# markusmoenig/Rusterix

Measured on AMD Instinct MI355X. Metric: Mpixels/s (+ ms/frame) on rasterize_map @3840x2160, 1/2/4/8 MI355X vs CPU, higher is better.
Workload: dtype f32; 1 GPU; map scene (minigame room), 3840x2160, 16 point lights, Nearest sampling, fence cut-outs, 2D logo rectangle; UV jitter absent in the reference snapshot; triangles_3d=27, light_math=relaxed

## Files before the change

### rusterix_amd/csrc/rxr_kernels.hip

```cpp
#ifndef RXR_JIT
#include <hip/hip_runtime.h>

#include <cstdlib>
#include <cstring>

#include "rxr_launch.h"
#include "rxr_route.h"
#endif

#define TS_DESC_VALID 0x80000000u

#include "rxr_device.h"
#include "rxr_exact_math.h"
#include "rxr_project.h"
#include "rxr_vm.h"

#ifndef RXR_VM_WAVES_PER_SIMD
#define RXR_VM_WAVES_PER_SIMD 6
#endif
#ifndef RXR_VEK_FUSED_MATVEC
#define RXR_VEK_FUSED_MATVEC 1
#endif

#ifndef RXR_PHASE_TIMING
// ... 312 lines not shown
    }
    return 1.0f;
}

__device__ __forceinline__ bool mapmini_is_visible(const rxr_linedef *ld, uint32_t n, float ax, float ay, float bx, float by) {
    for (uint32_t i = 0; i < n; ++i) {
        const rxr_linedef seg = uniform_record(ld, i);
        float b1x = seg.start[0], b1y = seg.start[1], b2x = seg.end[0], b2y = seg.end[1];
        float d = (bx - ax) * (b2y - b1y) - (by - ay) * (b2x - b1x);
        if (d == 0.0f) continue;
        float u = ((b1x - ax) * (b2y - b1y) - (b1y - ay) * (b2x - b1x)) / d;
        float v = ((b1x - ax) * (by - ay) - (b1y - ay) * (bx - ax)) / d;
        if ((u >= 0.0f && u <= 1.0f) && (v >= 0.0f && v <= 1.0f)) return false;
    }
    return true;
}

__device__ __forceinline__ uint32_t pack4(uint32_t r, uint32_t g, uint32_t b, uint32_t a) {
    return r | (g << 8) | (b << 16) | (a << 24);
}

__device__ __forceinline__ float grid_mul_dist(float delta, float value) {
    return fabsf(value - delta * roundf(value / delta));
}
__device__ __forceinline__ uint32_t grid_shade(const RasterParams &P, uint32_t px, uint32_t py) {
    const float grid = P.bg_grid[0], sub_div = P.bg_grid[1];
    const float pos_x = ((float)px / P.fwidth) * P.fwidth, pos_y = ((float)py / P.fheight) * P.fheight;
    const float origin_x = P.fwidth / 2.0f + P.bg_grid[2], origin_y = P.fheight / 2.0f + P.bg_grid[3];
    const float ao_x = roundf(origin_x - 0.5f) + 0.5f, ao_y = roundf(origin_y - 0.5f) + 0.5f;
    const float rel_x = pos_x - ao_x, rel_y = pos_y - ao_y;
    const float dist_x = grid_mul_dist(grid, rel_x), dist_y = grid_mul_dist(grid, rel_y);
    const uint32_t line = pack4(f32_to_u8_saturated(0.15f), f32_to_u8_saturated(0.15f), f32_to_u8_saturated(0.15f), f32_to_u8_saturated(1.0f));
    const uint32_t sub_line = pack4(f32_to_u8_saturated(0.11f), f32_to_u8_saturated(0.11f), f32_to_u8_saturated(0.11f), f32_to_u8_saturated(1.0f));
    const uint32_t bg = pack4(f32_to_u8_saturated(0.05f), f32_to_u8_saturated(0.05f), f32_to_u8_saturated(0.05f), f32_to_u8_saturated(1.0f));
    if (fminf(dist_x, dist_y) <= 1.0f * 0.5f) return line;
    const float dtf_x = fabsf(rel_x - grid * floorf(rel_x / grid)), dtf_y = fabsf(rel_y - grid * floorf(rel_y / grid));
    const float sub_size = grid / roundf(sub_div);
    float sd_x = grid_mul_dist(sub_size, dtf_x), sd_y = grid_mul_dist(sub_size, dtf_y);
    const float rc_x = roundf(dist_x / sub_size), rc_y = roundf(dist_y / sub_size);
    const float extra = grid - sub_size * sub_div;
    if (rc_x == sub_div) sd_x = sd_x + extra;
    if (rc_y == sub_div) sd_y = sd_y + extra;
    if (fminf(sd_x, sd_y) <= 1.0f * 0.5f) return sub_line;
    return bg;
}

__device__ __forceinline__ void fragment_uv(const TriShade &S, float alpha, float beta, float gamma, float &u, float &v) {
    float iu = S.u0w * alpha + S.u1w * beta + S.u2w * gamma;
    float iv = S.v0w * alpha + S.v1w * beta + S.v2w * gamma;
    float irw = S.iw0 * alpha + S.iw1 * beta + S.iw2 * gamma;
    rxm::div2(iu, iv, irw, u, v);
}

__device__ __forceinline__ const uint32_t *texel_base(const RasterParams &P, const DevTexDesc &d) {
    unsigned long long ft = (unsigned long long)P.frame_texels, rt = (unsigned long long)P.texels;
    asm volatile("" : "+v"(ft), "+v"(rt));
    typedef const uint32_t __attribute__((address_space(1))) *global_words;
    return (const uint32_t *)(global_words)((d.all_opaque & 2u) ? ft : rt);
}

__device__ __forceinline__ uint32_t terrain_texel(const RasterParams &P, const DevBatch &B, float wx, float wy) {
    const ChunkRange cr = P.chunks[B.chunk];
    const DevTexDesc d = P.tex[B.tex];
    float local_x = (wx / 1.0f) - (float)cr.origin_x;
    float local_y = (wy / 1.0f) - (float)cr.origin_y;
    float pixel_x = local_x * (float)cr.pixels_per_tile;
    float pixel_y = local_y * (float)cr.pixels_per_tile;
    uint32_t px = sat_u32(rclamp(floorf(pixel_x), 0.0f, (float)d.w - 1.0f));
    uint32_t py = sat_u32(rclamp(floorf(pixel_y), 0.0f, (float)d.h - 1.0f));
    px = min(px, d.w - 1u);
    py = min(py, d.h - 1u);
    return texel_base(P, d)[d.offset + py * d.w + px];
}

__device__ __forceinline__ float brush_blend(const RasterParams &P, f3 world, bool &inside) {
    const float dist = mag3(sub3(world, mk3(P.brush_pos[0], P.brush_pos[1], P.brush_pos[2])));
    inside = dist < P.brush_radius;
    const float normalized = dist / P.brush_radius;
    const float falloff = rclamp(P.brush_falloff, 0.001f, 1.0f);
    const float fade = rclamp((1.0f - normalized) / falloff, 0.0f, 1.0f);
    return 0.2f + 0.6f * fade;
}
__device__ __forceinline__ uint32_t brush_over_texel(const RasterParams &P, uint32_t texel, f3 world) {
    bool inside;
    const float blend = brush_blend(P, world, inside);
    if (!inside) return texel;
    uint32_t out = texel & 0xFF000000u;
#pragma unroll
    for (int i = 0; i < 3; ++i) {
        const float c = (float)((texel >> (8 * i)) & 0xFFu);
        out |= sat_u8(fminf(c * (1.0f - blend) + 255.0f * blend, 255.0f)) << (8 * i);
    }
    return out;
}

template <Level LV> inline constexpr LevelFeatures feat = level_features(LV);

template <Level LV, bool UNIFORM = false>
__device__ __forceinline__ uint32_t batch_texel(const RasterParams &P, const DevBatch &B, float u, float v, float wx, float wy, const f3 *world3 = nullptr) {
    if constexpr (!UNIFORM && !feat<LV>.chunk) {
        static_assert(__builtin_offsetof(DevBatch, tex) == 16 && __builtin_offsetof(DevBatch, pixel) == 20 && __builtin_offsetof(DevBatch, repeat_mode) == 24, "one 16-byte load");
        const uint4 hw = *reinterpret_cast<const uint4 *>(&B.tex);
        int32_t tex = (int32_t)hw.x;
        uint32_t pixel = hw.y, repeat = hw.z;
        asm volatile("" : "+v"(tex), "+v"(pixel), "+v"(repeat));
        if (tex < 0) return pixel;
        const uint4 raw = *reinterpret_cast<const uint4 *>(&P.tex[tex]);
        DevTexDesc d{raw.x, raw.y, raw.z, raw.w};
        asm volatile("" : "+v"(d.offset), "+v"(d.w), "+v"(d.h), "+v"(d.all_opaque));
        return sample_texture(d, texel_base(P, d), u, v, P.sample_mode, repeat);
    }
    if (B.tex < 0) return B.pixel;
    if constexpr (feat<LV>.chunk) {
        if (B.flags & DB_TERRAIN) {
            uint32_t t = terrain_texel(P, B, wx, wy);
            if (P.has_brush && world3) t = brush_over_texel(P, t, *world3);
            return t;
        }
    }
    if constexpr (UNIFORM) {
        const DevTexDesc d = uniform_record(P.tex, (uint32_t)B.tex);
        return sample_texture(d, texel_base(P, d), u, v, P.sample_mode, B.repeat_mode);
    } else {
        const uint4 raw = *reinterpret_cast<const uint4 *>(&P.tex[B.tex]);
        DevTexDesc d{raw.x, raw.y, raw.z, raw.w};
        asm volatile("" : "+v"(d.offset), "+v"(d.w), "+v"(d.h), "+v"(d.all_opaque));
        static_assert(sizeof(DevTexDesc) == 16, "one 16-byte load");
        return sample_texture(d, texel_base(P, d), u, v, P.sample_mode, B.repeat_mode);
    }
}

struct Frag {
    f3 world, normal, view_dir, base, lit;
    float opacity;
    uint32_t alpha_bits;
    float rough, metal;
    f3 emis;
};

__device__ __forceinline__ f3 screen_to_world_exact(const RasterParams &P, float fx, float fy, float z) {
    float vx, vy, vz, vw, wx, wy, wz, ww;
    const float x_ndc = 2.0f * rxm::div1_known(fx, P.fwidth, true) - 1.0f;
    const float y_ndc = 1.0f - 2.0f * rxm::div1_known(fy, P.fheight, true);
    mat4_mul(P.inv_proj, x_ndc, y_ndc, z, 1.0f, vx, vy, vz, vw);
    rxm::div3_self(vx, vy, vz, vw, vx, vy, vz, vw);
    mat4_mul(P.inv_view, vx, vy, vz, vw, wx, wy, wz, ww);
    return mk3(wx, wy, wz);
}

template <Level LV, bool RL = false>
__device__ __forceinline__ void shade3d_begin(const RasterParams &P, const TriShade &S, uint32_t batch_id, float alpha, float beta,
                                              float z, float fx, float fy, Frag &F, bool have_flags = false, uint32_t known_flags = 0u) {
    const DevBatch &B = P.batches3d[batch_id];
    const uint32_t b_flags = have_flags ? known_flags : B.flags;
    float gamma = 1.0f - alpha - beta;
    float u, v;
    fragment_uv(S, alpha, beta, gamma, u, v);

    bool relaxed_world = RL && !feat<LV>.chunk && !feat<LV>.programs && !P.any_occluders;
    f3 world;
    if (relaxed_world) {
        float vx, vy, vz, vw, wx, wy, wz, ww;
        mat4_mul(P.inv_proj, fmaf(fx, P.ndc_sx, -1.0f), fmaf(fy, P.ndc_sy, 1.0f), z, 1.0f, vx, vy, vz, vw);
        relaxed_world = rxm::wave_all(rxm::in_window(vw));
        if (relaxed_world) {
            const float rw = __builtin_amdgcn_rcpf(vw);
            mat4_mul(P.inv_view, vx * rw, vy * rw, vz * rw, 1.0f, wx, wy, wz, ww);
            world = mk3(wx, wy, wz);
        }
    }
    if (!relaxed_world) world = screen_to_world_exact(P, fx, fy, z);
    f3 cam = mk3(P.cam[0], P.cam[1], P.cam[2]);
    f3 view_dir, normal;
    bool relaxed_normals = false;
    if constexpr (RL && !feat<LV>.programs) {
        const bool has_n = (b_flags & DB_HAS_NORMALS) != 0u;
        const f3 vd = sub3(cam, world);
        f3 ni = mk3(0.0f, 0.0f, 0.0f);
        if (has_n) {
            f3 n0 = mk3(S.n0[0], S.n0[1], S.n0[2]), n1 = mk3(S.n1[0], S.n1[1], S.n1[2]), n2 = mk3(S.n2[0], S.n2[1], S.n2[2]);
            ni = add3(add3(scale3(n0, alpha), scale3(n1, beta)), scale3(n2, gamma));
        }
        const float vm2 = fmaf(vd.z, vd.z, fmaf(vd.y, vd.y, vd.x * vd.x)), nm2 = fmaf(ni.z, ni.z, fmaf(ni.y, ni.y, ni.x * ni.x));
        const float vinv = __builtin_amdgcn_rsqf(vm2), ninv = __builtin_amdgcn_rsqf(nm2);
        const float dnv = fmaf(ni.z, vd.z, fmaf(ni.y, vd.y, ni.x * vd.x)) * (vinv * ninv);
        float guard = P.rl_flip_guard;
        if (relaxed_world) guard = fmaf(1e-5f * vinv, __builtin_fabsf(world.x) + __builtin_fabsf(world.y) + __builtin_fabsf(world.z), guard);
        relaxed_normals = rxm::wave_all(rxm::sq_in_window(vm2) && (!has_n || (rxm::sq_in_window(nm2) && __builtin_fabsf(dnv) >= guard)));
        if (relaxed_normals) {
            view_dir = scale3(vd, vinv);
            normal = has_n ? scale3(ni, dnv < 0.0f ? -ninv : ninv) : mk3(__builtin_nanf(""), __builtin_nanf(""), __builtin_nanf(""));
        }
    }
    if (!relaxed_normals) {
        if (relaxed_world) world = screen_to_world_exact(P, fx, fy, z);
        view_dir = norm3_fast(sub3(cam, world));
        if (b_flags & DB_HAS_NORMALS) {
            f3 n0 = mk3(S.n0[0], S.n0[1], S.n0[2]), n1 = mk3(S.n1[0], S.n1[1], S.n1[2]), n2 = mk3(S.n2[0], S.n2[1], S.n2[2]);
            normal = norm3_z(add3(add3(scale3(n0, alpha), scale3(n1, beta)), scale3(n2, gamma)));
            if (dot3(normal, view_dir) < 0.0f) normal = neg3(normal);
        } else {
            normal = mk3(0.0f, 0.0f, 0.0f);
        }
    }

    uint32_t texel;
    bool desc_in_record = false;
    if constexpr (!feat<LV>.chunk || !feat<LV>.programs) desc_in_record = rxm::wave_all((S.pad[1] & TS_DESC_VALID) != 0u);
    if (desc_in_record) {
        const uint32_t p0 = S.pad[0], p1 = S.pad[1];
        const DevTexDesc d{p0, p1 & 0x1FFFu, (p1 >> 13) & 0x1FFFu, (p1 >> 28) & 3u};
        texel = sample_texture(d, texel_base(P, d), u, v, P.sample_mode, (p1 >> 26) & 3u);
    } else texel = batch_texel<LV>(P, B, u, v, world.x, world.z, &world);
    const float INV_255 = 1.0f / 255.0f;
    f3 base = mk3(srgb_to_linear_fast((float)(texel & 0xFFu) * INV_255), srgb_to_linear_fast((float)((texel >> 8) & 0xFFu) * INV_255),
                  srgb_to_linear_fast((float)((texel >> 16) & 0xFFu) * INV_255));
    F.opacity = rxm::div1_known((float)(texel >> 24), 255.0f, true);
    F.alpha_bits = texel & 0xFF000000u;
    if (feat<LV>.chunk && B.baked_plus1) {
        const DevTexDesc &baked = P.tex[B.baked_plus1 - 1u];
        uint32_t bt = sample_texture(baked, texel_base(P, baked), u, v, P.sample_mode, B.repeat_mode);
        base = mk3(srgb_to_linear_fast((float)(bt & 0xFFu) * INV_255), srgb_to_linear_fast((float)((bt >> 8) & 0xFFu) * INV_255),
                   srgb_to_linear_fast((float)((bt >> 16) & 0xFFu) * INV_255));
        F.opacity = (float)(bt >> 24) * INV_255;
    }
    float rough = 0.5f, metal = 0.0f;
    if constexpr (feat<LV>.programs) {
        if (B.program_plus1) {
            rxvm::IO io;
            rxvm::io_defaults(io);
            io.color = rxvm::mk(base.x, base.y, base.z);
            io.opacity.x = F.opacity;
            io.normal = rxvm::mk(normal.x, normal.y, normal.z);
            io.roughness.x = 0.5f;
            io.metallic.x = 0.0f;
            io.uv.x = u / 4.0f;
            io.uv.y = v / 4.0f;
            io.hitpoint = rxvm::mk(world.x, world.y, world.z);
            io.time = rxvm::splat(P.time);
            if constexpr (feat<LV>.inline_site) rxvm::shade_inline<feat<LV>.ssp>(P, B.program_plus1 - 1u, io, rxvm::stack_block());
            else rxvm::shade_call<feat<LV>.ssp>(P, B.program_plus1 - 1u, io);
            base = mk3(io.color.x, io.color.y, io.color.z);
            normal = mk3(io.normal.x, io.normal.y, io.normal.z);
            rough = rclamp(io.roughness.x, 0.0f, 1.0f);
            metal = rclamp(io.metallic.x, 0.0f, 1.0f);
            F.opacity = io.opacity.x;
            F.emis = mk3(io.emissive.x, io.emissive.y, io.emissive.z);
        }
    }

    if (!relaxed_normals) normal = norm3_z(normal);

    f3 lit = mk3(0.0f, 0.0f, 0.0f);
    float occlusion;
    static_assert(__builtin_offsetof(DevBatch, ambient) == 32 && __builtin_offsetof(DevBatch, chunk) == 44, "one 16-byte load");
    const uint4 amb_chunk = *reinterpret_cast<const uint4 *>(&B.ambient[0]);
    float amb0 = __uint_as_float(amb_chunk.x), amb1 = __uint_as_float(amb_chunk.y), amb2 = __uint_as_float(amb_chunk.z);
    int32_t b_chunk = (int32_t)amb_chunk.w;
    asm volatile("" : "+v"(amb0), "+v"(amb1), "+v"(amb2), "+v"(b_chunk));
    if (b_chunk >= 0) {
        ChunkRange cr = P.chunks[b_chunk];
        occlusion = get_occlusion(P.occluders, cr.occ_first, cr.occ_count, world.x, world.z);
    } else {
        occlusion = get_occlusion(P.occluders, 0, P.n_occluders, world.x, world.z);
    }
    float hemi = 0.5f * (normal.y + 1.0f);
    f3 kd = scale3(scale3(base, 1.0f - metal), 1.0f - 0.04f);
    if (occlusion > 0.0f) {
        if (P.flags & RXR_FLAG_HAS_AMBIENT) {
            lit = add3(lit, scale3(mul3(mk3(P.ambient[0], P.ambient[1], P.ambient[2]), kd), hemi));
        }
        if ((P.flags & RXR_FLAG_HAS_SUN) && P.day_factor > 0.0f) {
            f3 ldir = norm3(neg3(mk3(P.sun_dir[0], P.sun_dir[1], P.sun_dir[2])));
            float df = fmaxf(P.day_factor, 0.0f);
            lit = add3(lit, shade_fast_brdf(base, rough, metal, normal, view_dir, ldir, mk3(df, df, df), fmaxf(dot3(normal, ldir), 0.0f)));
        }
        lit = scale3(lit, occlusion);
    }
    lit = add3(lit, scale3(mul3(mk3(amb0, amb1, amb2), kd), hemi));
    F.world = world;
    F.normal = normal;
    F.view_dir = view_dir;
    F.base = base;
    F.lit = lit;
    F.rough = rough;
    F.metal = metal;
}

template <Level LV, bool RL = false>
__device__ __forceinline__ void shade3d_lights(const RasterParams &P, bool hit, Frag &F) {
    const unsigned long long hitmask = __ballot(hit);
    if (hitmask == 0ull) return;
    const int lane = (int)(threadIdx.x & 63u);
    const int src = __ffsll((long long)hitmask) - 1;
    const f3 c = mk3(__int_as_float(__builtin_amdgcn_readlane(__float_as_int(F.world.x), src)),
                     __int_as_float(__builtin_amdgcn_readlane(__float_as_int(F.world.y), src)),
                     __int_as_float(__builtin_amdgcn_readlane(__float_as_int(F.world.z), src)));
    const float r = hit ? mag3_bound(sub3(F.world, c)) : 0.0f;
    const bool can_cull = __ballot(hit && !(r < __builtin_huge_valf())) == 0ull;
    const float rmax = rxm::wave_max_nonneg(r);
    const float rough = feat<LV>.programs ? F.rough : 0.5f, metal = feat<LV>.programs ? F.metal : 0.0f;
    f3 rl_kd = mk3(0.0f, 0.0f, 0.0f), rl_f = rl_kd;
    float rl_shininess = 1.0f;
    if constexpr (RL && !feat<LV>.programs) {
        rl_kd = scale3(F.base, 1.0f - 0.04f);
        rl_shininess = 6.0f;
        const float om = 1.0f - rclamp(fmaxf(dot3(F.normal, F.view_dir), 0.0f), 0.0f, 1.0f);
        const float fs = 0.04f + (1.0f - 0.04f) * (om * om * om * om * om);
        rl_f = mk3(fs, fs, fs);
    } else if constexpr (RL) {
        const float tm = rclamp(metal, 0.0f, 1.0f);
        const f3 f0 = mk3(fmaf(tm, F.base.x - 0.04f, 0.04f), fmaf(tm, F.base.y - 0.04f, 0.04f), fmaf(tm, F.base.z - 0.04f, 0.04f));
        rl_kd = scale3(scale3(F.base, 1.0f - metal), 1.0f - fmaxf(f0.x, fmaxf(f0.y, f0.z)));
        rl_shininess = rclamp(2.0f / fmaxf(rough * rough, 1e-4f) - 2.0f, 1.0f, 2048.0f);
        const float om = 1.0f - rclamp(fmaxf(dot3(F.normal, F.view_dir), 0.0f), 0.0f, 1.0f);
        rl_f = add3(f0, scale3(sub3(mk3(1.0f, 1.0f, 1.0f), f0), om * om * om * om * om));
    }

    for (uint32_t base_i = 0; base_i < P.n_lights; base_i += 64u) {
        const uint32_t mine = base_i + (uint32_t)lane;
        bool cand = mine < P.n_lights;
        float ss_rcp = 0.0f;
        bool ss_ok = false;
        unsigned long long ss_ok_mask = 0ull;
        unsigned long long fast_mask = 0ull;
        if constexpr (RL) {
            bool fast = false;
            if (cand) {
                const float4 *lf4 = reinterpret_cast<const float4 *>(&P.lights_fast[mine]);
                const float4 head = lf4[0], tail = lf4[2];
                f3 lpos = mk3(head.x, head.y, head.z);
                float endd = tail.x;
                asm volatile("" : "+v"(lpos.x), "+v"(lpos.y), "+v"(lpos.z), "+v"(endd));
                const uint32_t kind = __float_as_uint(tail.y);
                fast = __float_as_uint(head.w) != 0u;
                if (can_cull && kind) {
                    float dcl = mag3_bound(sub3(c, lpos));
                    float margin = 1e-3f * (dcl + rmax + fabsf(endd)) + 1e-6f;
                    if (dcl - rmax > endd + margin) cand = false;
                }
            }
            fast_mask = __ballot(cand && fast);
            if (__ballot(cand && !fast)) {
                if (cand && !fast) {
                    const float ssd = P.lights[mine].start_distance - P.lights[mine].end_distance;
                    ss_ok = rxm::in_window(ssd);
                    ss_rcp = rxm::rcp_refined(ssd);
                }
                ss_ok_mask = __ballot(ss_ok);
            }
        } else {
            if (cand) {
                const float ssd = P.lights[mine].start_distance - P.lights[mine].end_distance;
                ss_ok = rxm::in_window(ssd);
                ss_rcp = rxm::rcp_refined(ssd);
            }
            ss_ok_mask = __ballot(ss_ok);
            if (cand && can_cull) {
                const rxr_light &L = P.lights[mine];
                if (L.light_type == RXR_LIGHT_POINT || L.light_type == RXR_LIGHT_SPOT || L.light_type == RXR_LIGHT_AREA ||
                    L.light_type == RXR_LIGHT_DAYLIGHT) {
                    float dcl = mag3_bound(sub3(c, mk3(L.position[0], L.position[1], L.position[2])));
                    float margin = 1e-3f * (dcl + rmax + fabsf(L.end_distance)) + 1e-6f;
                    if (dcl - rmax > L.end_distance + margin) cand = false;
                }
            }
        }
        unsigned long long todo = __ballot(cand);
        while (todo) {
            const int li_lane = __ffsll((long long)todo) - 1;
            const uint32_t li = base_i + (uint32_t)li_lane;
            todo &= todo - 1ull;
            float ss_r = 0.0f;
            bool ss_fast = false;
            if constexpr (!RL) {
                ss_r = __int_as_float(__builtin_amdgcn_readlane(__float_as_int(ss_rcp), li_lane));
                ss_fast = (ss_ok_mask >> li_lane) & 1ull;
            }
            if (!hit) continue;
            if constexpr (RL) {
                if ((fast_mask >> li_lane) & 1ull) {
                    const LightFast LF = uniform_record_x8(P.lights_fast, li);
                    const f3 d = sub3(mk3(LF.pos[0], LF.pos[1], LF.pos[2]), F.world);
                    const float m2 = fmaf(d.z, d.z, fmaf(d.y, d.y, d.x * d.x));
                    if (rxm::wave_all(rxm::sq_in_window(m2))) {
                        const float inv = __builtin_amdgcn_rsqf(m2);
                        const float t = __builtin_amdgcn_fmed3f(fmaf(m2 * inv, LF.ss_r, LF.c0), 0.0f, 1.0f);
                        const float ss = t * t * fmaf(-2.0f, t, 3.0f);
                        const float ndl = __builtin_amdgcn_fmed3f(fmaf(F.normal.z, d.z, fmaf(F.normal.y, d.y, F.normal.x * d.x)) * inv, 0.0f, 1.0f);
                        const f3 hu = mk3(fmaf(d.x, inv, F.view_dir.x), fmaf(d.y, inv, F.view_dir.y), fmaf(d.z, inv, F.view_dir.z));
                        const float hh = fmaf(hu.z, hu.z, fmaf(hu.y, hu.y, hu.x * hu.x));
                        const float ndh = __builtin_amdgcn_fmed3f(fmaf(F.normal.z, hu.z, fmaf(F.normal.y, hu.y, F.normal.x * hu.x)) * __builtin_amdgcn_rsqf(hh), 0.0f, 1.0f);
                        float spec;
                        if constexpr (!feat<LV>.programs) {
                            const float ndh2 = ndh * ndh;
                            spec = ndh2 * ndh2 * ndh2;
                        } else {
                            spec = __builtin_amdgcn_exp2f(rl_shininess * __builtin_amdgcn_logf(ndh));
                        }
                        const float s = ss * ndl * ndl;
                        F.lit.x = fmaf(fmaf(rl_f.x, spec, rl_kd.x), LF.cfi[0] * s, F.lit.x);
                        F.lit.y = fmaf(fmaf(rl_f.y, spec, rl_kd.y), LF.cfi[1] * s, F.lit.y);
                        F.lit.z = fmaf(fmaf(rl_f.z, spec, rl_kd.z), LF.cfi[2] * s, F.lit.z);
                        continue;
                    }
                }
            }
            if constexpr (RL) {
                ss_r = __int_as_float(__builtin_amdgcn_readlane(__float_as_int(ss_rcp), li_lane));
                ss_fast = (ss_ok_mask >> li_lane) & 1ull;
            }
            const rxr_light L = uniform_record(P.lights, li);
            const f3 lp = mk3(L.position[0], L.position[1], L.position[2]);
            f3 incoming, ldir;
            if (L.light_type == RXR_LIGHT_POINT) {
                if (!L.emitting) continue;
                f3 d = sub3(lp, F.world);
                float distance;
                ldir = norm3_fast(d, distance);
                if (distance >= L.end_distance) continue;
                float intensity = L.intensity;
                if (!(distance <= L.start_distance)) {
                    const float sn = distance - L.end_distance, sd = L.start_distance - L.end_distance;
                    float q;
                    if (ss_fast && rxm::wave_all(rxm::in_window(sn))) q = rxm::div_chain(sn, sd, ss_r);
                    else q = sn / sd;
                    const float t = rclamp(q, 0.0f, 1.0f);
                    intensity = L.intensity * (t * t * (3.0f - 2.0f * t));
                }
                incoming = apply_flicker(L, intensity, P.hash_anim);
            } else {
                if (!light_color_at(L, F.world, P.hash_anim, false, incoming)) continue;
                ldir = norm3_fast(sub3(lp, F.world));
            }
            const float n_dot_l = fmaxf(dot3(F.normal, ldir), 0.0f);
            f3 radiance;
            if (L.light_type == RXR_LIGHT_AMBIENT || L.light_type == RXR_LIGHT_AMBIENT_DAYLIGHT || L.light_type == RXR_LIGHT_DAYLIGHT) {
                radiance = incoming;
            } else {
                radiance = scale3(incoming, n_dot_l);
            }
            float rough_g = rough, metal_g = metal;
            if constexpr (RL) asm volatile("" : "+v"(rough_g), "+v"(metal_g));
            F.lit = add3(F.lit, shade_fast_brdf<RL>(F.base, rough_g, metal_g, F.normal, F.view_dir, ldir, radiance, n_dot_l));
        }
    }
}

template <Level LV, bool RL = false>
__device__ __forceinline__ uint32_t shade3d_end(const Frag &F) {
    f3 lit = F.lit;
    if constexpr (feat<LV>.programs) lit = add3(lit, F.emis);
    uint32_t alpha;
    if constexpr (feat<LV>.chunk || feat<LV>.programs) alpha = f32_to_u8_saturated(F.opacity) << 24;
    else alpha = F.alpha_bits;
    if constexpr (RL) {
        const float sx = __builtin_amdgcn_sqrtf(lit.x), sy = __builtin_amdgcn_sqrtf(lit.y), sz = __builtin_amdgcn_sqrtf(lit.z);
        return pack4(f32_to_u8_saturated(1.055f * sx - 0.055f * sx * sx), f32_to_u8_saturated(1.055f * sy - 0.055f * sy * sy),
                     f32_to_u8_saturated(1.055f * sz - 0.055f * sz * sz), 0u) | alpha;
    }
    return pack4(f32_to_u8_saturated(linear_to_srgb_fast(lit.x)), f32_to_u8_saturated(linear_to_srgb_fast(lit.y)),
                 f32_to_u8_saturated(linear_to_srgb_fast(lit.z)), 0u) | alpha;
}

template <Level LV>
__device__ __forceinline__ uint32_t shade3d_opacity(const RasterParams &P, const TriShade &S, uint32_t batch_id, float alpha, float beta,
                                                    float z, float fx, float fy) {
    const DevBatch &B = P.batches3d[batch_id];
    float gamma = 1.0f - alpha - beta;
    float u, v;
    fragment_uv(S, alpha, beta, gamma, u, v);
    float wx = 0.0f, wy = 0.0f, wz = 0.0f;
    if ((feat<LV>.chunk && (B.flags & DB_TERRAIN)) || (feat<LV>.programs && B.program_plus1)) {
        float x_ndc = 2.0f * (fx / P.fwidth) - 1.0f;
        float y_ndc = 1.0f - 2.0f * (fy / P.fheight);
        float vx, vy, vz, vw, ww;
        mat4_mul(P.inv_proj, x_ndc, y_ndc, z, 1.0f, vx, vy, vz, vw);
        vx = vx / vw;
        vy = vy / vw;
        vz = vz / vw;
        vw = vw / vw;
        mat4_mul(P.inv_view, vx, vy, vz, vw, wx, wy, wz, ww);
    }
    const f3 world3 = mk3(wx, wy, wz);
    uint32_t texel = batch_texel<LV>(P, B, u, v, wx, wz, &world3);
    const float INV_255 = 1.0f / 255.0f;
    float r = srgb_to_linear_fast((float)(texel & 0xFFu) * INV_255);
    float g = srgb_to_linear_fast((float)((texel >> 8) & 0xFFu) * INV_255);
    float b = srgb_to_linear_fast((float)((texel >> 16) & 0xFFu) * INV_255);
    float opacity = byte_over_255(texel >> 24);
    if constexpr (feat<LV>.programs) {
        if (B.program_plus1) {
            rxvm::IO io;
            rxvm::io_defaults(io);
            io.color = rxvm::mk(r, g, b);
            io.opacity.x = opacity;
            io.uv.x = u / 4.0f;
            io.uv.y = v / 4.0f;
            io.hitpoint = rxvm::mk(wx, wy, wz);
            io.time = rxvm::splat(P.time);
            io.roughness.x = 0.5f;
            io.metallic.x = 0.0f;
            rxvm::shade_call<feat<LV>.ssp>(P, B.program_plus1 - 1u, io);
            r = io.color.x;
            g = io.color.y;
            b = io.color.z;
            opacity = io.opacity.x;
        }
    }
    return pack4(f32_to_u8_saturated(linear_to_srgb_fast(r)), f32_to_u8_saturated(linear_to_srgb_fast(g)),
                 f32_to_u8_saturated(linear_to_srgb_fast(b)), f32_to_u8_saturated(opacity));
}

template <Level LV>
__device__ __forceinline__ uint32_t fragment2d(const RasterParams &P, const Prim2D &T, const DevBatch &B, uint32_t px, uint32_t py,
                                               float fx, float fy, uint32_t dst) {
    float acx = T.v2x - T.v0x, acy = T.v2y - T.v0y;
    float abx = T.v1x - T.v0x, aby = T.v1y - T.v0y;
    float apx = fx - T.v0x, apy = fy - T.v0y;
    float pcx = T.v2x - fx, pcy = T.v2y - fy;
    float pbx = T.v1x - fx, pby = T.v1y - fy;
    float area = acx * aby - acy * abx;
    float w0 = (pcx * pby - pcy * pbx) / area;
    float w1 = (acx * apy - acy * apx) / area;
    float w2 = 1.0f - w0 - w1;
    float u = T.u0 * w0 + T.u1 * w1 + T.u2 * w2;
    float v = T.v0 * w0 + T.v1 * w1 + T.v2 * w2;

    float gx = ((float)px - P.fwidth / 2.0f) - (P.translationd2[0] - P.fwidth / 2.0f);
    float gy = ((float)py - P.fheight / 2.0f) - (P.translationd2[1] - P.fheight / 2.0f);
    float wx = gx / P.scaled2, wy = gy / P.scaled2;

    uint32_t texel = batch_texel<LV, true>(P, B, u, v, wx, wy);
    if constexpr (feat<LV>.programs) {
        if (B.program_plus1 && P.programs[B.program_plus1 - 1u].shade_entry != 0xFFFFFFFFu) {
            const float INV_255 = 1.0f / 255.0f;
            rxvm::IO io;
            rxvm::io_defaults(io);
            io.uv.x = u / 4.0f;
            io.uv.y = v / 4.0f;
            io.color = rxvm::mk((float)(texel & 0xFFu) * INV_255, (float)((texel >> 8) & 0xFFu) * INV_255, (float)((texel >> 16) & 0xFFu) * INV_255);
            io.hitpoint.x = wx;
            io.hitpoint.y = wy;
            io.time = rxvm::splat(P.time);
            io.roughness.x = 0.5f;
            io.metallic.x = 0.0f;
            rxvm::shade_call<feat<LV>.ssp>(P, B.program_plus1 - 1u, io);
            texel = pack4(f32_to_u8_saturated(io.color.x), f32_to_u8_saturated(io.color.y), f32_to_u8_saturated(io.color.z), 255u);
        }
    }
    uint32_t tr = texel & 0xFFu, tg = (texel >> 8) & 0xFFu, tb = (texel >> 16) & 0xFFu, ta = texel >> 24;

    if (((B.flags & DB_RECEIVES_LIGHT) && P.any_lights) || (P.flags & RXR_FLAG_HAS_AMBIENT)) {
        float acc0 = 0.0f, acc1 = 0.0f, acc2 = 0.0f;
        uint32_t occ_first = 0, occ_count = P.n_occluders;
        if (B.chunk >= 0) {
            ChunkRange cr = P.chunks[B.chunk];
            occ_first = cr.occ_first;
            occ_count = cr.occ_count;
        }
        if (P.flags & RXR_FLAG_HAS_AMBIENT) {
            float occlusion = get_occlusion(P.occluders, occ_first, occ_count, wx, wy);
            acc0 += P.ambient[0] * occlusion;
            acc1 += P.ambient[1] * occlusion;
            acc2 += P.ambient[2] * occlusion;
        }
        for (uint32_t li = 0; li < P.n_lights; ++li) {
            const rxr_light L = uniform_record(P.lights, li);
            f3 lc;
            if (!light_color_at(L, mk3(wx, 0.0f, wy), P.hash_anim, true, lc)) continue;
            bool visible = true;
            if (L.light_type == RXR_LIGHT_AMBIENT_DAYLIGHT) {
                float occlusion = get_occlusion(P.occluders, occ_first, occ_count, wx, wy);
                lc = scale3(lc, occlusion);
            }
            if (L.light_type != RXR_LIGHT_AMBIENT && L.light_type != RXR_LIGHT_AMBIENT_DAYLIGHT &&
                !mapmini_is_visible(P.linedefs, P.n_linedefs, wx, wy, L.position[0], L.position[2]))
                visible = false;
            if (visible) {
                acc0 += lc.x;
                acc1 += lc.y;
                acc2 += lc.z;
            }
        }
        acc0 = rclamp(acc0, 0.0f, 1.0f);
        acc1 = rclamp(acc1, 0.0f, 1.0f);
        acc2 = rclamp(acc2, 0.0f, 1.0f);
        tr = sat_u8(rclamp((byte_over_255(tr) * acc0) * 255.0f, 0.0f, 255.0f));
        tg = sat_u8(rclamp((byte_over_255(tg) * acc1) * 255.0f, 0.0f, 255.0f));
        tb = sat_u8(rclamp((byte_over_255(tb) * acc2) * 255.0f, 0.0f, 255.0f));
    }

    if (ta == 255u) return pack4(tr, tg, tb, ta);
    float src_alpha = byte_over_255(ta);
    float dst_alpha = 1.0f - src_alpha;
    uint32_t dr = dst & 0xFFu, dg = (dst >> 8) & 0xFFu, db = (dst >> 16) & 0xFFu, da = dst >> 24;
    uint32_t orr = sat_u8(((float)tr * src_alpha) + ((float)dr * dst_alpha));
    uint32_t og = sat_u8(((float)tg * src_alpha) + ((float)dg * dst_alpha));
    uint32_t ob = sat_u8(((float)tb * src_alpha) + ((float)db * dst_alpha));
    uint32_t oa = (P.flags & RXR_FLAG_PRESERVE_TRANSPARENCY) ? max(da, ta) : 255u;
    return pack4(orr, og, ob, oa);
}

__device__ __forceinline__ uint32_t miss_brush_preview(const RasterParams &P, uint32_t px, uint32_t py) {
    const float ndc_x = 2.0f * ((float)px / P.fwidth) - 1.0f;
    const float ndc_y = 1.0f - 2.0f * ((float)py / P.fheight);
    float nx, ny, nz, nw, fx_, fy_, fz_, fw_;
    mat4_mul(P.inv_proj, ndc_x, ndc_y, -1.0f, 1.0f, nx, ny, nz, nw);
    mat4_mul(P.inv_proj, ndc_x, ndc_y, 1.0f, 1.0f, fx_, fy_, fz_, fw_);
    nx = nx / nw; ny = ny / nw; nz = nz / nw; nw = nw / nw;
    fx_ = fx_ / fw_; fy_ = fy_ / fw_; fz_ = fz_ / fw_; fw_ = fw_ / fw_;
    float ox, oy, oz, ow, tx, ty, tz, tw;
    mat4_mul(P.inv_view, nx, ny, nz, nw, ox, oy, oz, ow);
    mat4_mul(P.inv_view, fx_, fy_, fz_, fw_, tx, ty, tz, tw);
    const f3 origin = mk3(ox, oy, oz);
    const f3 dir = norm3(sub3(mk3(tx, ty, tz), origin));
    float c = 0.0f;
    if (fabsf(dir.y) > 1e-5f) {
        const float t = -origin.y / dir.y;
        if (t > 0.0f) {
            bool inside;
            const float blend = brush_blend(P, add3(origin, scale3(dir, t)), inside);
            if (inside) c = fminf(0.0f * (1.0f - blend) + blend, 1.0f);
        }
    }
    const uint32_t g = f32_to_u8_saturated(c);
    return pack4(g, g, g, f32_to_u8_saturated(1.0f));
}

__device__ __forceinline__ bool bin_range(const RasterParams &P, uint32_t min_x, uint32_t max_x, uint32_t min_y, uint32_t max_y,
                                          uint32_t &bx0, uint32_t &bx1, uint32_t &l0, uint32_t &l1) {
    if (!(min_x < max_x && min_y < max_y) || P.tiles_y == 0) return false;
    bx0 = min_x / RXR_TILE_W;
    bx1 = (max_x - 1) / RXR_TILE_W;
    uint32_t g0 = min_y / RXR_TILE_H, g1 = (max_y - 1) / RXR_TILE_H;
    if (g1 < P.tile_y0) return false;
    l0 = g0 <= P.tile_y0 ? 0u : (g0 - P.tile_y0 + P.tile_stride - 1u) / P.tile_stride;
    l1 = (g1 - P.tile_y0) / P.tile_stride;
    if (l1 >= P.tiles_y) l1 = P.tiles_y - 1u;
    return l0 <= l1;
}

__device__ __forceinline__ bool make_setup(const RasterParams &P, uint32_t t, TriSetup &S, TriShade &H) {
    uint32_t lo = 0, hi = P.n_batches3d;
    const bool have_info = P.tri_info != nullptr;
    uint2 info = make_uint2(0u, 0u);
    if (have_info) {
        info = P.tri_info[t];
        lo = info.x;
    } else {
        while (hi - lo > 1) {
            uint32_t mid = (lo + hi) >> 1;
            if (P.batch_tri_base[mid] <= t) lo = mid;
            else hi = mid;
        }
    }
    if (P.mesh_live && t - P.batch_tri_base[lo] >= P.mesh_live[lo]) {
        S.bx = S.by = 0u;
        return false;
    }
    const bool own_edges = P.pm_meshes != nullptr;
    const bool host_edgeless = P.edge_vis3d != nullptr;
    rxr_edges E;
    if (!own_edges && !host_edgeless) E = P.edges[t];
    const uint32_t ix0 = P.idx[3 * (size_t)t + 0], ix1 = P.idx[3 * (size_t)t + 1], ix2 = P.idx[3 * (size_t)t + 2];
    const DevBatch B = P.batches3d[lo];
    const uint32_t vbase = have_info ? info.y : B.vert_base;
    if (own_edges) {
        const DevMesh &M = P.pm_meshes[lo];
        const uint32_t local = t - P.batch_tri_base[lo];
        const bool evis = local < M.n_tris ? P.pm_edge_vis[M.tin_base + local] != 0 : true;
        E = edges_from_vertices(M.cull_mode, evis, P.pv[ix0 + vbase], P.pv[ix1 + vbase], P.pv[ix2 + vbase]);
    } else if (host_edgeless) {
        E = edges_from_vertices(B.mode, P.edge_vis3d[t] != 0u, P.pv[ix0 + vbase], P.pv[ix1 + vbase], P.pv[ix2 + vbase]);
    }

    bool skip = (B.flags & DB_SKIP) != 0;
    if (P.dev_bbox) {
        const DevBBox bb = P.dev_bbox[lo];
        auto dec = [](uint32_t e) { return __uint_as_float((e & 0x80000000u) ? (e ^ 0x80000000u) : ~e); };
        float bx = dec(bb.min_x), by = dec(bb.min_y), bw = dec(bb.max_x) - bx, bh = dec(bb.max_y) - by;
        bool keep = bx < (float)P.width && (bx + bw) > 0.0f && by < (float)P.height && (by + bh) > 0.0f;
        skip = skip || !keep;
    }
    if (!E.visible || skip) {
        S.bx = S.by = 0u;
        return false;
    }

    const uint32_t i0 = ix0 + vbase, i1 = ix1 + vbase, i2 = ix2 + vbase;
    float4 v0 = P.pv[i0], v1 = P.pv[i1], v2 = P.pv[i2];

#pragma unroll
    for (int k = 0; k < 3; ++k) {
        S.ea[k] = E.a[k];
        S.eb[k] = E.b[k];
        S.ec[k] = E.c[k];
    }
    S.v0x = v0.x; S.v0y = v0.y; S.v1x = v1.x; S.v1y = v1.y; S.v2x = v2.x; S.v2y = v2.y;
    {
        float acx = v2.x - v0.x, acy = v2.y - v0.y, abx = v1.x - v0.x, aby = v1.y - v0.y;
        S.area = acx * aby - acy * abx;
    }
    S.iz0 = 1.0f / v0.z;
    S.iz1 = 1.0f / v1.z;
    S.iz2 = 1.0f / v2.z;
    S.batch = lo;
    S.bflags = B.flags;
    S.profile_id = B.profile_id;

    H.iw0 = 1.0f / v0.w;
    H.iw1 = 1.0f / v1.w;
    H.iw2 = 1.0f / v2.w;
    float2 uv0 = P.uv[i0], uv1 = P.uv[i1], uv2 = P.uv[i2];
    H.u0w = uv0.x / v0.w; H.u1w = uv1.x / v1.w; H.u2w = uv2.x / v2.w;
    H.v0w = uv0.y / v0.w; H.v1w = uv1.y / v1.w; H.v2w = uv2.y / v2.w;
    if (B.flags & DB_HAS_NORMALS) {
#pragma unroll
        for (int k = 0; k < 3; ++k) {
            H.n0[k] = P.nrm[3 * (size_t)i0 + k];
            H.n1[k] = P.nrm[3 * (size_t)i1 + k];
            H.n2[k] = P.nrm[3 * (size_t)i2 + k];
        }
    } else {
#pragma unroll
        for (int k = 0; k < 3; ++k) H.n0[k] = H.n1[k] = H.n2[k] = 0.0f;
    }
    H.pad[0] = H.pad[1] = 0;
    if (B.tex >= 0 && !(B.flags & DB_TERRAIN) && B.repeat_mode < 4u) {
        const DevTexDesc d = P.tex[B.tex];
        if (d.w - 1u < 8191u && d.h - 1u < 8191u) {
            H.pad[0] = d.offset;
            H.pad[1] = TS_DESC_VALID | d.w | (d.h << 13) | (B.repeat_mode << 26) | ((d.all_opaque & 3u) << 28);
        }
    }
    if (P.sample_mode != RXR_SAMPLE_NEAREST && B.tex >= 0 && !(S.bflags & (DB_ALPHA_TEST | DB_FULL_ALPHA | DB_OPACITY_LIST))) {
        const float t9[9] = {H.iw0, H.iw1, H.iw2, H.u0w, H.u1w, H.u2w, H.v0w, H.v1w, H.v2w};
        bool risky = false;
#pragma unroll
        for (int k = 0; k < 9; ++k) risky = risky || !(__builtin_fabsf(t9[k]) < __builtin_huge_valf());
        const float lo = fminf(__builtin_fabsf(H.iw0), fminf(__builtin_fabsf(H.iw1), __builtin_fabsf(H.iw2)));
        const float hi = fmaxf(__builtin_fabsf(H.iw0), fmaxf(__builtin_fabsf(H.iw1), __builtin_fabsf(H.iw2)));
        const bool same_sign = (H.iw0 > 0.0f && H.iw1 > 0.0f && H.iw2 > 0.0f) || (H.iw0 < 0.0f && H.iw1 < 0.0f && H.iw2 < 0.0f);
        risky = risky || !same_sign || !(hi <= lo * 1048576.0f);
#ifndef RXR_TEST_NO_NAN_UV_RULE
        if (risky) S.bflags |= DB_ALPHA_TEST;
#endif
    }
// ... 2102 lines not shown
```

Measured before the change: 75590 Mpixels/s.

## Factor fast-light BRDF into deferred diffuse/specular sums and simplify half-vector math

Fast point lights now add their terms into separate diffuse and specular sums, and the material coefficients are applied once after the light loop. The half-vector length is computed algebraically from n·v and d·v instead of forming the half vector. A per-light 'sure' mask skips the wave-wide range check when a conservative bound already guarantees it, and that check now only considers hit lanes. This removes per-light multiplies and a ballot on the hot path. In exchange it adds registers for the accumulators and changes rounding order slightly.

```diff
diff --git a/rusterix_amd/csrc/rxr_kernels.hip b/rusterix_amd/csrc/rxr_kernels.hip
--- a/rusterix_amd/csrc/rxr_kernels.hip
+++ b/rusterix_amd/csrc/rxr_kernels.hip
@@ -638,10 +638,12 @@
     const float rough = feat<LV>.programs ? F.rough : 0.5f, metal = feat<LV>.programs ? F.metal : 0.0f;
     f3 rl_kd = mk3(0.0f, 0.0f, 0.0f), rl_f = rl_kd;
     float rl_shininess = 1.0f;
+    float rl_nv = 0.0f;
+    if constexpr (RL) rl_nv = dot3(F.normal, F.view_dir);
     if constexpr (RL && !feat<LV>.programs) {
         rl_kd = scale3(F.base, 1.0f - 0.04f);
         rl_shininess = 6.0f;
-        const float om = 1.0f - rclamp(fmaxf(dot3(F.normal, F.view_dir), 0.0f), 0.0f, 1.0f);
+        const float om = 1.0f - rclamp(fmaxf(rl_nv, 0.0f), 0.0f, 1.0f);
         const float fs = 0.04f + (1.0f - 0.04f) * (om * om * om * om * om);
         rl_f = mk3(fs, fs, fs);
     } else if constexpr (RL) {
@@ -649,9 +651,11 @@
         const f3 f0 = mk3(fmaf(tm, F.base.x - 0.04f, 0.04f), fmaf(tm, F.base.y - 0.04f, 0.04f), fmaf(tm, F.base.z - 0.04f, 0.04f));
         rl_kd = scale3(scale3(F.base, 1.0f - metal), 1.0f - fmaxf(f0.x, fmaxf(f0.y, f0.z)));
         rl_shininess = rclamp(2.0f / fmaxf(rough * rough, 1e-4f) - 2.0f, 1.0f, 2048.0f);
-        const float om = 1.0f - rclamp(fmaxf(dot3(F.normal, F.view_dir), 0.0f), 0.0f, 1.0f);
+        const float om = 1.0f - rclamp(fmaxf(rl_nv, 0.0f), 0.0f, 1.0f);
         rl_f = add3(f0, scale3(sub3(mk3(1.0f, 1.0f, 1.0f), f0), om * om * om * om * om));
     }
+    f3 rl_sum_d = mk3(0.0f, 0.0f, 0.0f), rl_sum_s = rl_sum_d;
+    bool rl_summed = false;
 
     for (uint32_t base_i = 0; base_i < P.n_lights; base_i += 64u) {
         const uint32_t mine = base_i + (uint32_t)lane;
@@ -660,8 +664,9 @@
         bool ss_ok = false;
         unsigned long long ss_ok_mask = 0ull;
         unsigned long long fast_mask = 0ull;
+        unsigned long long sure_mask = 0ull;
         if constexpr (RL) {
-            bool fast = false;
+            bool fast = false, sure = false;
             if (cand) {
                 const float4 *lf4 = reinterpret_cast<const float4 *>(&P.lights_fast[mine]);
                 const float4 head = lf4[0], tail = lf4[2];
@@ -674,9 +679,11 @@
                     float dcl = mag3_bound(sub3(c, lpos));
                     float margin = 1e-3f * (dcl + rmax + fabsf(endd)) + 1e-6f;
                     if (dcl - rmax > endd + margin) cand = false;
+                    sure = dcl - rmax > margin && dcl + rmax < 0x1p39f;
                 }
             }
             fast_mask = __ballot(cand && fast);
+            sure_mask = __ballot(cand && fast && sure);
             if (__ballot(cand && !fast)) {
                 if (cand && !fast) {
                     const float ssd = P.lights[mine].start_distance - P.lights[mine].end_distance;
@@ -713,20 +720,21 @@
                 ss_r = __int_as_float(__builtin_amdgcn_readlane(__float_as_int(ss_rcp), li_lane));
                 ss_fast = (ss_ok_mask >> li_lane) & 1ull;
             }
-            if (!hit) continue;
+            bool general = true;
             if constexpr (RL) {
                 if ((fast_mask >> li_lane) & 1ull) {
                     const LightFast LF = uniform_record_x8(P.lights_fast, li);
                     const f3 d = sub3(mk3(LF.pos[0], LF.pos[1], LF.pos[2]), F.world);
                     const float m2 = fmaf(d.z, d.z, fmaf(d.y, d.y, d.x * d.x));
-                    if (rxm::wave_all(rxm::sq_in_window(m2))) {
+                    if (((sure_mask >> li_lane) & 1ull) || (__builtin_amdgcn_ballot_w64(!rxm::sq_in_window(m2)) & hitmask) == 0ull) {
                         const float inv = __builtin_amdgcn_rsqf(m2);
                         const float t = __builtin_amdgcn_fmed3f(fmaf(m2 * inv, LF.ss_r, LF.c0), 0.0f, 1.0f);
                         const float ss = t * t * fmaf(-2.0f, t, 3.0f);
-                        const float ndl = __builtin_amdgcn_fmed3f(fmaf(F.normal.z, d.z, fmaf(F.normal.y, d.y, F.normal.x * d.x)) * inv, 0.0f, 1.0f);
-                        const f3 hu = mk3(fmaf(d.x, inv, F.view_dir.x), fmaf(d.y, inv, F.view_dir.y), fmaf(d.z, inv, F.view_dir.z));
-                        const float hh = fmaf(hu.z, hu.z, fmaf(hu.y, hu.y, hu.x * hu.x));
-                        const float ndh = __builtin_amdgcn_fmed3f(fmaf(F.normal.z, hu.z, fmaf(F.normal.y, hu.y, F.normal.x * hu.x)) * __builtin_amdgcn_rsqf(hh), 0.0f, 1.0f);
+                        const float nd = fmaf(F.normal.z, d.z, fmaf(F.normal.y, d.y, F.normal.x * d.x));
+                        const float ndl = __builtin_amdgcn_fmed3f(nd * inv, 0.0f, 1.0f);
+                        const float dv = fmaf(F.view_dir.z, d.z, fmaf(F.view_dir.y, d.y, F.view_dir.x * d.x));
+                        const float hh = fmaf(dv * inv, 2.0f, 2.0f);
+                        const float ndh = __builtin_amdgcn_fmed3f(fmaf(nd, inv, rl_nv) * __builtin_amdgcn_rsqf(hh), 0.0f, 1.0f);
                         float spec;
                         if constexpr (!feat<LV>.programs) {
                             const float ndh2 = ndh * ndh;
@@ -735,13 +743,15 @@
                             spec = __builtin_amdgcn_exp2f(rl_shininess * __builtin_amdgcn_logf(ndh));
                         }
                         const float s = ss * ndl * ndl;
-                        F.lit.x = fmaf(fmaf(rl_f.x, spec, rl_kd.x), LF.cfi[0] * s, F.lit.x);
-                        F.lit.y = fmaf(fmaf(rl_f.y, spec, rl_kd.y), LF.cfi[1] * s, F.lit.y);
-                        F.lit.z = fmaf(fmaf(rl_f.z, spec, rl_kd.z), LF.cfi[2] * s, F.lit.z);
-                        continue;
+                        const float sp = s * spec;
+                        rl_sum_d = mk3(fmaf(LF.cfi[0], s, rl_sum_d.x), fmaf(LF.cfi[1], s, rl_sum_d.y), fmaf(LF.cfi[2], s, rl_sum_d.z));
+                        rl_sum_s = mk3(fmaf(LF.cfi[0], sp, rl_sum_s.x), fmaf(LF.cfi[1], sp, rl_sum_s.y), fmaf(LF.cfi[2], sp, rl_sum_s.z));
+                        rl_summed = true;
+                        general = false;
                     }
                 }
             }
+            if (!general || !hit) continue;
             if constexpr (RL) {
                 ss_r = __int_as_float(__builtin_amdgcn_readlane(__float_as_int(ss_rcp), li_lane));
                 ss_fast = (ss_ok_mask >> li_lane) & 1ull;
@@ -780,6 +790,11 @@
             if constexpr (RL) asm volatile("" : "+v"(rough_g), "+v"(metal_g));
             F.lit = add3(F.lit, shade_fast_brdf<RL>(F.base, rough_g, metal_g, F.normal, F.view_dir, ldir, radiance, n_dot_l));
         }
+    }
+    if (RL && rl_summed) {
+        F.lit.x = fmaf(rl_f.x, rl_sum_s.x, fmaf(rl_kd.x, rl_sum_d.x, F.lit.x));
+        F.lit.y = fmaf(rl_f.y, rl_sum_s.y, fmaf(rl_kd.y, rl_sum_d.y, F.lit.y));
+        F.lit.z = fmaf(rl_f.z, rl_sum_s.z, fmaf(rl_kd.z, rl_sum_d.z, F.lit.z));
     }
 }
 
```

New measurement: 75620 Mpixels/s, median of 2. About the same (+0.0%).
